# zachdedoo13/compute_path_tracer

Hardware: AMD Instinct MI355X
Metric: Msamples/sec at 1920×1080×8-bounce; achieved HBM GB/s vs gfx950 peak (higher is better)
Workload: dtype f32; 1 GPU; c3 1920x1080, 8 bounces, 256 spp per step (256 per GPU-share), progressive accumulate; width=1920, height=1080, bounces=8, parallelism=tiles1, pipelines=2, bin_samples=536870912, bin_fallback=False

## Files before the change

compute_path_tracer_amd/csrc/pt_binned.h:

```cpp
#pragma once

#include "pt_path.h"

#ifndef PT_BIN_BITS
#define PT_BIN_BITS 12
#endif
#define PT_BINS (1 << PT_BIN_BITS)
#define PT_BIN_NONE 0xffffffffu
#define PT_AUX_MISS 0xffffffffu
#define PT_BIN_BLOCK 256
#ifndef PT_RUN_SHARDS
#define PT_RUN_SHARDS 8
#endif
#define PT_CTRL_CURSOR(k) (32u * (1u + uint32_t(k)))
#define PT_CTRL_STRIDE (32u * (1u + uint32_t(PT_RUN_SHARDS)))
#ifndef PT_SCATTER_ITEMS
#define PT_SCATTER_ITEMS 16
#endif

struct PtRay {
    uint4 q[4];
};

struct PtPass {
    PtLaunch L;
    PtRay *rin;
    PtRay *rout;
    uint4 *hq;
    uint2 *mask_hi;
    uint32_t *key;
    uint32_t *idx;
    uint32_t *hist;
    uint32_t *offs;
    uint32_t *ctrl;
    const uint32_t *n_src;
    float4 *color;
    float4 *hitn;
    unsigned long long *btab;
    int32_t lanes;
    uint32_t n_src_const;
    int32_t bounce;
    int32_t n_pix;
    int32_t frames;
    int32_t wide;
    int32_t run_max;
    int32_t refill_min;
    int32_t gen_order;
    int32_t gen_trace;
    int32_t count_overflow;
    int32_t gen_norec;
};

namespace pt {

__device__ __forceinline__ uint32_t bin_hash(const uint4 &m) {
    const uint32_t h = (m.x * 0x9E3779B1u) ^ (m.y * 0x85EBCA77u) ^ (m.z * 0xC2B2AE3Du) ^ (m.w * 0x27D4EB2Fu);
    return (h ^ (h >> 15)) * 0x2C1B3C6Du >> (32 - PT_BIN_BITS);
}

#ifndef PT_BIN_PROBES
#define PT_BIN_PROBES 8
#endif
struct BinProbe {
    uint32_t h;
    unsigned long long e;
    unsigned long long v;
};
__device__ __forceinline__ BinProbe bin_probe(const PtPass &P, const uint4 &m) {
    BinProbe b;
    b.h = bin_hash(m);
    b.e = 0ull;
    b.v = 0ull;
    if (P.btab) {
        b.e = ((unsigned long long)m.y << 32 | m.x) + 1ull;
        if (b.e != 0ull) b.v = P.btab[b.h];
    }
    return b;
}
__device__ __forceinline__ uint32_t bin_resolve(const PtPass &P, const uint4 &m, BinProbe b) {
    if (!P.btab) {
        if ((m.y | m.z | m.w) == 0u && m.x < uint32_t(PT_BINS)) return m.x;
        return b.h;
    }
    if (b.e == 0ull || b.v == b.e) return b.h;
    uint32_t s = b.h;
    unsigned long long v = b.v;
    for (int k = 0;;) {
        if (v == 0ull) v = atomicCAS(P.btab + s, 0ull, b.e);
        if (v == 0ull || v == b.e) return s;
        if (++k == PT_BIN_PROBES) {
            if (P.count_overflow) atomicAdd(P.btab + PT_BINS, 1ull);
            return b.h;
        }
        s = (s + 1u) & uint32_t(PT_BINS - 1);
        v = P.btab[s];
    }
}

template <bool ST>
__device__ __forceinline__ uint4 bounds_mask(const PtLaunch &L, const pt_f3 &ro, const pt_f3 &rd, Stats<ST> &st) {
    uint32_t w[4] = {0u, 0u, 0u, 0u};
    const caabb_ptr boxes = (caabb_ptr)L.aabbs;
    const bool fast = L.fast_bounds != 0 && pt_div_coord_ok(ro.x) && pt_div_coord_ok(ro.y) &&
                      pt_div_coord_ok(ro.z) && pt_div_dir_ok(rd.x) && pt_div_dir_ok(rd.y) && pt_div_dir_ok(rd.z);
    if (fast) {
        if constexpr (ST)
            if (first_active_lane()) st.add(PT_ST_BOUNDS_WAVES);
        const float yx = 1.0f / rd.x, yy = 1.0f / rd.y, yz = 1.0f / rd.z;
        uint32_t gapu = 0xffffffffu;
#pragma unroll 4
        for (int b = 0; b < L.n_aabb; ++b) {
            const PtAabb bx = boxes[b];
            if (ray_box_ulp<false>(bx, ro.x, ro.y, ro.z, yx, yy, yz, gapu)) w[bx.back >> 5] |= 1u << (bx.back & 31);
        }
        if (__builtin_expect(__ballot(!(gapu > PT_ULP_MARGIN)) != 0ull, 0)) {
            if constexpr (ST)
                if (first_active_lane()) st.add(PT_ST_BOUNDS_EXACT);
            uint32_t v[4] = {0u, 0u, 0u, 0u};
            for (int b = 0; b < L.n_aabb; ++b) {
                const PtAabb bx = boxes[b];
                if (ray_box_rcp(bx, ro.x, ro.y, ro.z, rd.x, rd.y, rd.z, yx, yy, yz))
                    v[bx.back >> 5] |= 1u << (bx.back & 31);
            }
            if (!(gapu > PT_ULP_MARGIN))
                for (int k = 0; k < 4; ++k) w[k] = v[k];
        }
    } else {
        for (int b = 0; b < L.n_aabb; ++b) {
            const PtAabb bx = boxes[b];
            if (ray_box(bx, ro.x, ro.y, ro.z, rd.x, rd.y, rd.z)) w[bx.back >> 5] |= 1u << (bx.back & 31);
        }
    }
    st.add(PT_ST_SEGMENTS);
    st.add(PT_ST_AABB, uint32_t(L.n_aabb));
    return make_uint4(w[0], w[1], w[2], w[3]);
}

template <class Map>
struct MapWide {
    static constexpr int v = -1;
};
template <class Map>
__device__ __forceinline__ bool wide_of(const PtPass &P) {
    if constexpr (MapWide<Map>::v >= 0) return MapWide<Map>::v != 0;
    else return P.wide != 0;
}

template <class Map>
struct MapMats {
    static constexpr int n = 0;
};

template <class Map>
struct MapBounds {
    template <bool ST>
    static __device__ __forceinline__ uint4 mask(const PtLaunch &L, const pt_f3 &ro, const pt_f3 &rd, Stats<ST> &st) {
        return bounds_mask<ST>(L, ro, rd, st);
    }
    template <bool ST>
    static __device__ __forceinline__ uint4 mask_skip(const PtLaunch &L, const pt_f3 &ro, const pt_f3 &rd, uint64_t skip,
                                                      Stats<ST> &st) {
        (void)skip;
        return bounds_mask<ST>(L, ro, rd, st);
    }
};

__device__ __forceinline__ uint64_t primary_box_skip(const PtLaunch &L, const pt_f3 &ro, const pt_f3 &rd) {
    const int nb = L.n_aabb;
    if (L.fast_bounds == 0 || nb <= 0 || nb > 64) return 0ull;
    if (__builtin_amdgcn_read_exec() != ~0ull) return 0ull;
    const bool fast = pt_div_coord_ok(ro.x) && pt_div_coord_ok(ro.y) && pt_div_coord_ok(ro.z) &&
                      pt_div_dir_ok(rd.x) && pt_div_dir_ok(rd.y) && pt_div_dir_ok(rd.z);
    const uint64_t fm = __ballot(fast);
    if (fm == 0ull) return 0ull;
    const int l0 = __builtin_ctzll(fm);
    const float ox = __int_as_float(__builtin_amdgcn_readlane(__float_as_int(ro.x), l0));
    const float oy = __int_as_float(__builtin_amdgcn_readlane(__float_as_int(ro.y), l0));
    const float oz = __int_as_float(__builtin_amdgcn_readlane(__float_as_int(ro.z), l0));
    if (__ballot(fast && (__float_as_uint(ro.x) != __float_as_uint(ox) || __float_as_uint(ro.y) != __float_as_uint(oy) ||
                          __float_as_uint(ro.z) != __float_as_uint(oz))) != 0ull)
        return 0ull;
    const float inf = __builtin_inff();
    const uint32_t lane = threadIdx.x & 63u;
    const bool mine = lane < uint32_t(nb);
    static_assert(sizeof(PtAabb) == 32, "box stride");
    uint32_t off;
    __asm__ volatile("v_lshlrev_b32 %0, 5, %1" : "=v"(off) : "v"(lane));
    const float *box = reinterpret_cast<const float *>(reinterpret_cast<const char *>(L.aabbs) + off);
    float lo = -inf, hi = inf;
    auto axis = [&](int a, float d, float o) {
        const float y = 1.0f / d;
        const float ylo = wave_min_f32(fast ? y : inf), yhi = wave_max_f32(fast ? y : -inf);
        if (mine && (ylo > 0.0f || yhi < 0.0f)) {
            const float c1 = box[a] - o, c2 = box[3 + a] - o;
            const float p1 = c1 * ylo, p2 = c1 * yhi, p3 = c2 * ylo, p4 = c2 * yhi;
            lo = pt_gmax(lo, pt_gmin(pt_gmin(p1, p2), pt_gmin(p3, p4)));
            hi = pt_gmin(hi, pt_gmax(pt_gmax(p1, p2), pt_gmax(p3, p4)));
        }
    };
    axis(0, rd.x, ox);
    axis(1, rd.y, oy);
    axis(2, rd.z, oz);
    const bool skip = mine && (hi <= 0.0f ||
                               (lo > 0.0f && hi > 0.0f && __float_as_uint(lo) > __float_as_uint(hi) + PT_ULP_MARGIN));
    return __ballot(skip);
}

__device__ __forceinline__ void store_ray(PtRay *r, const pt_f3 &ro, const pt_f3 &rd, const pt_f3 &thr, uint32_t rng,
                                          uint32_t sid, uint32_t aux, const uint4 &q3) {
    r->q[0] = make_uint4(__float_as_uint(ro.x), __float_as_uint(ro.y), __float_as_uint(ro.z), __float_as_uint(rd.x));
    r->q[1] = make_uint4(__float_as_uint(rd.y), __float_as_uint(rd.z), __float_as_uint(thr.x), __float_as_uint(thr.y));
    r->q[2] = make_uint4(__float_as_uint(thr.z), rng, sid, aux);
    r->q[3] = q3;
}

__device__ __forceinline__ void hist_zero(uint32_t *lh) {
    for (int b = int(threadIdx.x); b < PT_BINS; b += int(blockDim.x)) lh[b] = 0u;
    __syncthreads();
}
__device__ __forceinline__ void hist_flush(const uint32_t *lh, uint32_t *hist) {
    __syncthreads();
    for (int b = int(threadIdx.x); b < PT_BINS; b += int(blockDim.x))
        if (lh[b] != 0u) atomicAdd(&hist[b], lh[b]);
}
__device__ __forceinline__ void pixel_of(int rank, int nranks, int tiles_x, uint32_t pl, int &x, int &y) {
    const int k = int(pl >> 6), p = int(pl & 63u);
    const int g = rank + k * nranks;
    x = (g % tiles_x) * PT_TILE + (p & 7);
    y = (g / tiles_x) * PT_TILE + (p >> 3);
}
__device__ __forceinline__ void pixel_of(const PtLaunch &L, uint32_t pl, int &x, int &y) {
    pixel_of(L.rank, L.nranks, L.tiles_x, pl, x, y);
}
__device__ __forceinline__ void gen_sample(uint32_t frames, uint32_t p, uint32_t &f, uint32_t &pl) {
    pl = p / frames;
    f = p - pl * frames;
}
__device__ __forceinline__ uint32_t colour_slot(uint32_t frames, uint32_t f, uint32_t pl) { return pl * frames + f; }

template <class Map, bool ST, int CAM = PT_CAMK_ANY>
__device__ __forceinline__ void bin_gen_body(const PtPass &P) {
    __shared__ uint32_t lh[PT_BINS];
    hist_zero(lh);
    Stats<ST> st;
    st.init();
    const PtLaunch &L = P.L;
    const uint32_t npix = uint32_t(P.n_pix), n = npix * uint32_t(P.frames);
    for (uint32_t i = blockIdx.x * blockDim.x + threadIdx.x; i < n; i += gridDim.x * blockDim.x) {
        const uint32_t f = i / npix, pl = i - f * npix;
        int x, y;
        pixel_of(L, pl, x, y);
        const bool live = x < L.width && y < L.height;
        if (P.gen_order) P.idx[i] = i;
        if (!live) {
            if (!P.gen_order) P.key[i] = PT_BIN_NONE;
            continue;
        }
        uint32_t rng;
        pt_f3 ro, rd;
        camera_ray<CAM>(x, y, int32_t(uint32_t(L.frame0) + f), L.width, L.height, L.aspect, L.fov, L.cam_mode, L.cam,
                        rng, ro, rd);
        st.add(PT_ST_SAMPLES);
        const uint4 m = MapBounds<Map>::template mask<ST>(L, ro, rd, st);
        const BinProbe bp = P.gen_order ? BinProbe{0u, 0ull, 0ull} : bin_probe(P, m);
        const uint32_t sid = colour_slot(uint32_t(P.frames), f, pl);
        store_ray(P.rin + i, ro, rd, pt_f3{1.0f, 1.0f, 1.0f}, rng, sid, i, make_uint4(m.x, m.y, 0u, 0u));
        P.color[sid] = make_float4(0.0f, 0.0f, 0.0f, 0.0f);
        if (wide_of<Map>(P)) P.mask_hi[i] = make_uint2(m.z, m.w);
        if (!P.gen_order) {
            const uint32_t b = bin_resolve(P, m, bp);
            P.key[i] = b;
            atomicAdd(&lh[b], 1u);
        }
    }
    if (!P.gen_order) hist_flush(lh, P.hist);
    flush_stats<ST>(L, st);
}

template <class Map, bool ST, bool TAPS, int CAM = PT_CAMK_ANY>
__device__ __forceinline__ void bin_shade_body(const PtPass &P) {
    __shared__ uint32_t lh[PT_BINS];
    constexpr int NM = MapMats<Map>::n;
    __shared__ PtMat lm[NM > 0 ? NM : 1];
    const PtMat *mats = P.L.mats;
    if constexpr (NM > 0) {
        const uint4 *src = reinterpret_cast<const uint4 *>(P.L.mats);
        uint4 *dst = reinterpret_cast<uint4 *>(lm);
        for (int k = int(threadIdx.x); k < NM * int(sizeof(PtMat) / 16); k += int(blockDim.x)) dst[k] = src[k];
        mats = lm;
    }
    hist_zero(lh);
    Stats<ST> st;
    st.init();
    Stats<ST> stt;
    stt.init();
    const PtLaunch &L = P.L;
    const uint32_t n = P.n_src ? *P.n_src : P.n_src_const;
    auto shade_one = [&](uint32_t i, const uint4 &q0, const uint4 &q1, const uint4 &q2, const uint4 &q3,
                         const uint2 &hi, const uint4 &hq) {
        pt_f3 ro{__uint_as_float(q0.x), __uint_as_float(q0.y), __uint_as_float(q0.z)};
        pt_f3 rd{__uint_as_float(q0.w), __uint_as_float(q1.x), __uint_as_float(q1.y)};
        pt_f3 thr{__uint_as_float(q1.z), __uint_as_float(q1.w), __uint_as_float(q2.x)};
        pt_f3 ret{0.0f, 0.0f, 0.0f};
        uint32_t rng = q2.y;
        const uint32_t sid = q2.z;
        const int mat = int(TAPS ? q2.w : hq.y);
        int seg = P.bounce;
        float dv0 = __uint_as_float(q3.x), dv1 = __uint_as_float(q3.y), dv2 = __uint_as_float(q3.z);
        if constexpr (!TAPS) {
            const float t = __uint_as_float(hq.x);
            ro = pt_f3{ro.x + rd.x * t, ro.y + rd.y * t, ro.z + rd.z * t};
            Check ck{uint64_t(q3.x) | (uint64_t(q3.y) << 32), uint64_t(hi.x) | (uint64_t(hi.y) << 32)};
            const float bnd = __uint_as_float(hq.z);
            const float bndw = bnd + (0x1.a3ap-13f + 0x1p-20f * (fabsf(ro.x) + fabsf(ro.y) + fabsf(ro.z)));
            uint64_t live = 0ull;
            float dp = 0.0f;
#pragma unroll 1
            for (int k = 0; k < 6; ++k) {
                float qx, qy, qz;
                map_point(ST_NORMAL, k, ro, rd, 0.0f, qx, qy, qz);
                if constexpr (ST)
                    if (first_active_lane()) stt.add(PT_ST_WAVE_MAPS);
                const Hit h = k == 0 ? Map::template first<ST>(L, qx, qy, qz, ck, bnd, bndw, live, stt)
                                     : Map::template rest<ST>(L, qx, qy, qz, ck, bnd, bndw, live, stt);
                if (k == 0) ck.alo = Map::alive(live);
                if ((k & 1) == 0) {
                    dp = h.d;
                } else {
                    const float dd = dp - h.d;
                    if (k == 1) dv0 = dd;
                    else if (k == 3) dv1 = dd;
                    else dv2 = dd;
                }
            }
            stt.add(PT_ST_NORMAL_MAPS, 6);
        }
        const bool done = shade_lane<ST>(mats, L.bounces, mat, dv0, dv1, dv2, 0, rng, ro, rd, thr, ret, seg, st);
        if (P.bounce == 0) st.add(PT_ST_SHADED_FIRST);
        if (P.gen_trace) {
            P.color[sid] = make_float4(ret.x, ret.y, ret.z, 0.0f);
        } else if (ret.x != 0.0f || ret.y != 0.0f || ret.z != 0.0f) {
            float4 c = P.color[sid];
            c.x += ret.x;
            c.y += ret.y;
            c.z += ret.z;
            P.color[sid] = c;
        }
        if (done) {
            if (L.debug == 3) {
                const pt_f3 col = final_color(L.debug, seg, L.bounces, ret);
                P.color[sid] = make_float4(col.x, col.y, col.z, 0.0f);
            }
            P.key[i] = PT_BIN_NONE;
            return;
        }
        const uint4 m = MapBounds<Map>::template mask<ST>(L, ro, rd, st);
        const BinProbe bp = bin_probe(P, m);
        store_ray(P.rout + i, ro, rd, thr, rng, sid, i, make_uint4(m.x, m.y, 0u, 0u));
        if (wide_of<Map>(P)) P.mask_hi[i] = make_uint2(m.z, m.w);
        const uint32_t k = bin_resolve(P, m, bp);
        P.key[i] = k;
        atomicAdd(&lh[k], 1u);
    };
    for (uint32_t i = blockIdx.x * blockDim.x + threadIdx.x; i < n; i += gridDim.x * blockDim.x) {
        if constexpr (TAPS) {
            const uint4 q0 = P.rout[i].q[0], q1 = P.rout[i].q[1], q2 = P.rout[i].q[2], q3 = P.rout[i].q[3];
            if (q2.w == PT_AUX_MISS) P.key[i] = PT_BIN_NONE;
            else shade_one(i, q0, q1, q2, q3, make_uint2(0u, 0u), q3);
        } else {
            uint4 hq = P.hq[i];
            __asm__ volatile("" : "+v"(hq.x), "+v"(hq.y), "+v"(hq.z), "+v"(hq.w));
            if (hq.y == PT_AUX_MISS) {
                P.key[i] = PT_BIN_NONE;
                continue;
            }
            uint4 q0, q1, q2, q3;
            if (P.gen_norec) {
                uint32_t npix = uint32_t(P.n_pix), nf = uint32_t(P.frames);
                int rk = L.rank, nr = L.nranks, tx = L.tiles_x, cw = L.width, chh = L.height;
                float ca = L.aspect, cf = L.fov;
                __asm__ volatile("" : "+s"(npix), "+s"(nf), "+s"(rk), "+s"(nr), "+s"(tx), "+s"(cw), "+s"(chh),
                                 "+s"(ca), "+s"(cf));
                uint32_t f, pl;
                gen_sample(nf, i, f, pl);
                int x, y;
                pixel_of(rk, nr, tx, pl, x, y);
                uint32_t rg;
                pt_f3 o, d;
                camera_ray<CAM>(x, y, int32_t(uint32_t(L.frame0) + f), cw, chh, ca, cf, L.cam_mode, L.cam, rg, o, d);
                q0 = make_uint4(__float_as_uint(o.x), __float_as_uint(o.y), __float_as_uint(o.z), __float_as_uint(d.x));
                q1 = make_uint4(__float_as_uint(d.y), __float_as_uint(d.z), __float_as_uint(1.0f), __float_as_uint(1.0f));
                q2 = make_uint4(__float_as_uint(1.0f), rg, colour_slot(nf, f, pl), i);
                q3 = make_uint4(hq.w, 0u, 0u, 0u);
            } else {
                const PtRay *r = P.rin + hq.w;
                q0 = r->q[0];
                q1 = r->q[1];
                q2 = r->q[2];
                q3 = r->q[3];
            }
            uint2 hi = make_uint2(0u, 0u);
            if (wide_of<Map>(P)) {
                const float4 nd = P.hitn[i];
                hi = make_uint2(__float_as_uint(nd.z), __float_as_uint(nd.w));
            }
            shade_one(i, q0, q1, q2, q3, hi, hq);
        }
    }
    hist_flush(lh, P.hist);
    flush_stats<ST>(L, st);
    if constexpr (!TAPS) flush_stats<ST>(L, stt, PT_ST_COUNT);
}

#define PT_SCAN_THREADS 64
__device__ __forceinline__ void bin_scan_body(const PtPass &P) {
    constexpr int PER = PT_BINS / PT_SCAN_THREADS;
    const int t = int(threadIdx.x);
    uint4 *h4 = reinterpret_cast<uint4 *>(P.hist + t * PER);
    uint4 *o4 = reinterpret_cast<uint4 *>(P.offs + t * PER);
    uint32_t sum = 0u;
#pragma unroll
    for (int j = 0; j < PER / 4; ++j) {
        const uint4 v = h4[j];
        sum += v.x + v.y + v.z + v.w;
    }
    uint32_t inc = sum;
#pragma unroll
    for (int off = 1; off < PT_SCAN_THREADS; off <<= 1) {
        const uint32_t x = uint32_t(__shfl_up(int(inc), off, PT_SCAN_THREADS));
        if (t >= off) inc += x;
    }
    uint32_t run = inc - sum;
#pragma unroll
    for (int j = 0; j < PER / 4; ++j) {
        const uint4 v = h4[j];
        uint4 o;
        o.x = run;
        run += v.x;
        o.y = run;
        run += v.y;
        o.z = run;
        run += v.z;
        o.w = run;
        run += v.w;
        o4[j] = o;
        h4[j] = make_uint4(0u, 0u, 0u, 0u);
    }
    if (t == PT_SCAN_THREADS - 1) P.ctrl[0] = inc;
    if (t < PT_RUN_SHARDS) P.ctrl[PT_CTRL_CURSOR(t)] = 0u;
}

__device__ __forceinline__ void bin_scatter_body(const PtPass &P) {
    __shared__ uint32_t cnt[PT_BINS];
    const uint32_t n = P.n_src ? *P.n_src : P.n_src_const;
    const uint32_t per = ((n + gridDim.x - 1u) / gridDim.x + PT_BIN_BLOCK - 1u) & ~uint32_t(PT_BIN_BLOCK - 1);
    const uint32_t b0 = min(n, blockIdx.x * per), b1 = min(n, b0 + per);
    constexpr uint32_t U = 8u;
    hist_zero(cnt);
    for (uint32_t e0 = b0 + threadIdx.x; e0 < b1; e0 += U * PT_BIN_BLOCK) {
        uint32_t k[U];
#pragma unroll
        for (uint32_t j = 0; j < U; ++j) {
            const uint32_t e = e0 + j * PT_BIN_BLOCK;
            k[j] = e < b1 ? P.key[e] : PT_BIN_NONE;
        }
#pragma unroll
        for (uint32_t j = 0; j < U; ++j)
            if (k[j] != PT_BIN_NONE) atomicAdd(&cnt[k[j]], 1u);
    }
    __syncthreads();
    for (int b = int(threadIdx.x); b < PT_BINS; b += PT_BIN_BLOCK) {
        const uint32_t c = cnt[b];
        if (c != 0u) cnt[b] = atomicAdd(&P.offs[b], c);
    }
    __syncthreads();
    for (uint32_t e0 = b0 + threadIdx.x; e0 < b1; e0 += U * PT_BIN_BLOCK) {
        uint32_t k[U];
#pragma unroll
        for (uint32_t j = 0; j < U; ++j) {
            const uint32_t e = e0 + j * PT_BIN_BLOCK;
            k[j] = e < b1 ? P.key[e] : PT_BIN_NONE;
        }
#pragma unroll
        for (uint32_t j = 0; j < U; ++j)
            if (k[j] != PT_BIN_NONE) P.idx[atomicAdd(&cnt[k[j]], 1u)] = e0 + j * PT_BIN_BLOCK;
    }
}

template <class Map, bool ST, bool TAPS = true, bool GEN = false, int CAM = PT_CAMK_ANY>
__device__ __forceinline__ void bin_trace_body(const PtPass &P) {
    __shared__ uint4 W[MapWide<Map>::v == 0 ? 4 : 5][64];
    const PtLaunch &L = P.L;
    const int lane = int(threadIdx.x);
    Stats<ST> st;
    st.init();
    const uint64_t t_start = st.clk();
    const uint32_t n = P.ctrl[0];
    const uint32_t rmax = uint32_t(P.run_max);
    uint32_t R = n / (gridDim.x * 8u);
    R = R < 64u ? 64u : (R > rmax ? rmax : (R + 63u) & ~63u);
    uint32_t shard = blockIdx.x % PT_RUN_SHARDS, tried = 0u;
    auto shard_lo = [&](uint32_t k) -> uint32_t {
        return k >= PT_RUN_SHARDS ? n : uint32_t((uint64_t(n >> 6) * k / PT_RUN_SHARDS) << 6);
    };
    auto take = [&](uint32_t len, uint32_t &end) -> uint32_t {
        while (tried < PT_RUN_SHARDS) {
            const uint32_t lo = shard_lo(shard), hi = shard_lo(shard + 1u);
            const uint32_t b = lo + atomicAdd(&P.ctrl[PT_CTRL_CURSOR(shard)], len);
            if (b < hi) {
                end = b + len < hi ? b + len : hi;
                return b;
            }
            shard = (shard + 1u) % PT_RUN_SHARDS;
            ++tried;
        }
        end = n;
        return n;
    };

    uint32_t nxt = 0u, nxt_end = 0u;
    if (lane == 0) nxt = take(R, nxt_end);
    uint32_t run_cur = uint32_t(__builtin_amdgcn_readfirstlane(int(nxt)));
    uint32_t run_end = uint32_t(__builtin_amdgcn_readfirstlane(int(nxt_end)));
    if (lane == 0 && run_cur < n) nxt = take(R, nxt_end);
    auto next_window = [&](uint32_t &b, uint32_t &c) {
        if (run_cur >= run_end) {
            run_cur = uint32_t(__builtin_amdgcn_readfirstlane(int(nxt)));
            run_end = uint32_t(__builtin_amdgcn_readfirstlane(int(nxt_end)));
            if (lane == 0 && run_cur < n) nxt = take(R, nxt_end);
        }
        b = run_cur;
        c = run_end - run_cur < 64u ? run_end - run_cur : 64u;
        run_cur += c;
    };
    uint32_t nb = 0u, nc = 0u, nslot = 0u;
    next_window(nb, nc);
    if (!GEN && uint32_t(lane) < nc) nslot = P.idx[nb + uint32_t(lane)];
    uint32_t wbase = 0u, wcnt = 0u, wtake = 0u;
    float4 s0 = make_float4(0.0f, 0.0f, 0.0f, 0.0f), s1 = s0, s2 = s0;
    uint4 s3 = make_uint4(0u, 0u, 0u, 0u);
    uint2 sh = make_uint2(0u, 0u);
    bool in_lds = false;
    auto stage = [&]() {
        wbase = nb;
        wcnt = nc;
        wtake = 0u;
        in_lds = false;
        if (GEN && uint32_t(lane) < wcnt) {
            const uint32_t i = wbase + uint32_t(lane), npix = uint32_t(P.n_pix);
            uint32_t f, pl;
            gen_sample(uint32_t(P.frames), i, f, pl);
            const uint32_t sid = colour_slot(uint32_t(P.frames), f, pl);
            (void)npix;
            int x, y;
            pixel_of(L, pl, x, y);
            uint32_t rg;
            pt_f3 o, d;
            float fov = L.fov;
            __asm__ volatile("" : "+v"(fov));
            camera_ray<CAM>(x, y, int32_t(uint32_t(L.frame0) + f), L.width, L.height, L.aspect, fov, L.cam_mode, L.cam,
                            rg, o, d);
            st.add(PT_ST_SAMPLES);
            const uint64_t skip = wcnt == 64u ? primary_box_skip(L, o, d) : 0ull;
            const uint4 m = MapBounds<Map>::template mask_skip<ST>(L, o, d, skip, st);
            s0 = make_float4(o.x, o.y, o.z, d.x);
            s1 = make_float4(d.y, d.z, 1.0f, 1.0f);
            s2 = make_float4(1.0f, __uint_as_float(rg), __uint_as_float(sid), __uint_as_float(i));
            s3 = make_uint4(m.x, m.y, 0u, 0u);
            sh = make_uint2(m.z, m.w);
        } else if (uint32_t(lane) < wcnt) {
            const uint32_t slot = nslot;
            const uint4 *v = reinterpret_cast<const uint4 *>(P.rin + slot);
            const uint4 a = v[0], b = v[1], c = v[2];
            s0 = make_float4(__uint_as_float(a.x), __uint_as_float(a.y), __uint_as_float(a.z), __uint_as_float(a.w));
            s1 = make_float4(__uint_as_float(b.x), __uint_as_float(b.y), __uint_as_float(b.z), __uint_as_float(b.w));
            s2 = make_float4(__uint_as_float(c.x), __uint_as_float(c.y), __uint_as_float(c.z), __uint_as_float(c.w));
            s3 = v[3];
            if (wide_of<Map>(P)) sh = P.mask_hi[slot];
        }
        if (wcnt != 0u) {
            next_window(nb, nc);
            if (!GEN && uint32_t(lane) < nc) nslot = P.idx[nb + uint32_t(lane)];
        }
    };
    stage();

    int state = ST_FREE;
    uint32_t rng = 0u, sid = 0u, pos = 0u, slot = 0u;
    pt_f3 ro{0.0f, 0.0f, 0.0f}, rd{0.0f, 0.0f, 1.0f};
    pt_f3 thr{1.0f, 1.0f, 1.0f};
    int step = 0, mat = 0;
    float t = 0.0f;
    float dv0 = 0.0f, dv1 = 0.0f, dv2 = 0.0f;
    Check ck{0ull, 0ull};

    auto hand_on = [&]() {
        if (state == ST_SHADE) {
            if (step < 0) {
                if (L.debug == 3) {
                    const pt_f3 c = final_color(L.debug, P.bounce, L.bounces, pt_f3{0.0f, 0.0f, 0.0f});
                    P.color[sid] = make_float4(c.x, c.y, c.z, 0.0f);
                }
                if constexpr (TAPS) P.rout[pos].q[2] = make_uint4(slot, 0u, sid, PT_AUX_MISS);
                else P.hq[pos] = make_uint4(0u, PT_AUX_MISS, 0u, slot);
                if constexpr (GEN) P.color[sid] = make_float4(0.0f, 0.0f, 0.0f, 0.0f);
            } else {
                if constexpr (TAPS) {
                    store_ray(P.rout + pos, ro, rd, thr, rng, sid, uint32_t(mat),
                              make_uint4(__float_as_uint(dv0), __float_as_uint(dv1), __float_as_uint(dv2), 0u));
                } else {
                    P.hq[pos] = make_uint4(__float_as_uint(t), uint32_t(mat), __float_as_uint(dv0),
                                           GEN && P.gen_norec ? uint32_t(ck.lo) : slot);
                    if (wide_of<Map>(P))
                        P.hitn[pos] = make_float4(0.0f, 0.0f, __uint_as_float(uint32_t(ck.hi)),
                                                  __uint_as_float(uint32_t(ck.hi >> 32)));
                }
            }
            state = ST_FREE;
        }
    };

    auto park = [&]() {
        const bool mapping_now = state == ST_MARCH || (TAPS && state == ST_NORMAL);
        const bool in_win = uint32_t(lane) < wcnt;
        ck.alo = wave_or_u64((mapping_now ? ck.lo : 0ull) |
                             (in_win ? (uint64_t(s3.x) | (uint64_t(s3.y) << 32)) : 0ull));
        ck.ahi = wide_of<Map>(P) ? wave_or_u64((mapping_now ? ck.hi : 0ull) |
                                      (in_win ? (uint64_t(sh.x) | (uint64_t(sh.y) << 32)) : 0ull))
                        : 0ull;
        W[0][lane] = make_uint4(__float_as_uint(s0.x), __float_as_uint(s0.y), __float_as_uint(s0.z),
                                __float_as_uint(s0.w));
        W[1][lane] = make_uint4(__float_as_uint(s1.x), __float_as_uint(s1.y), __float_as_uint(s1.z),
                                __float_as_uint(s1.w));
        W[2][lane] = make_uint4(__float_as_uint(s2.x), __float_as_uint(s2.y), __float_as_uint(s2.z),
                                __float_as_uint(s2.w));
        W[3][lane] = s3;
        if constexpr (MapWide<Map>::v != 0)
            if (wide_of<Map>(P)) W[4][lane] = make_uint4(sh.x, sh.y, 0u, 0u);
        if constexpr (GEN) {
            if (in_win && !P.gen_norec) {
                uint4 *r = reinterpret_cast<uint4 *>(P.rin + wbase + uint32_t(lane));
                r[0] = make_uint4(__float_as_uint(s0.x), __float_as_uint(s0.y), __float_as_uint(s0.z),
                                  __float_as_uint(s0.w));
                r[1] = make_uint4(__float_as_uint(s1.x), __float_as_uint(s1.y), __float_as_uint(s1.z),
                                  __float_as_uint(s1.w));
                r[2] = make_uint4(__float_as_uint(s2.x), __float_as_uint(s2.y), __float_as_uint(s2.z),
                                  __float_as_uint(s2.w));
                r[3] = s3;
            }
        }
        in_lds = true;
        __builtin_amdgcn_fence(__ATOMIC_RELEASE, "wavefront");
        __builtin_amdgcn_wave_barrier();
        __builtin_amdgcn_fence(__ATOMIC_ACQUIRE, "wavefront");
    };

    for (;;) {
        uint64_t tm = st.clk();
        const uint64_t freem = __ballot(state == ST_FREE);
        if (freem != 0ull && wcnt != 0u &&
            (__popcll(freem) >= P.refill_min || __ballot(state == ST_MARCH || state == ST_NORMAL) == 0ull)) {
            const uint32_t avail = wcnt - wtake, nf = uint32_t(__popcll(freem));
            const uint32_t take = nf < avail ? nf : avail;
            const int r = lane_rank(freem);
            const int src = int(wtake) + r;
            const bool got = state == ST_FREE && uint32_t(r) < take;
            if (!in_lds) park();
            float a0 = 0.0f, a1 = 0.0f, a2 = 0.0f, a3 = 0.0f, b0 = 0.0f, b1 = 0.0f, b2 = 0.0f, b3 = 0.0f;
            float c0 = 0.0f, c1 = 0.0f, c2 = 0.0f, c3 = 0.0f;
            uint32_t d0 = 0u, d1 = 0u, d2 = 0u, d3 = 0u, e0 = 0u, e1 = 0u;
            if (got) {
                const uint4 wa = W[0][src], wb = W[1][src], wc = W[2][src], wd = W[3][src];
                a0 = __uint_as_float(wa.x), a1 = __uint_as_float(wa.y), a2 = __uint_as_float(wa.z);
                a3 = __uint_as_float(wa.w);
                b0 = __uint_as_float(wb.x), b1 = __uint_as_float(wb.y), b2 = __uint_as_float(wb.z);
                b3 = __uint_as_float(wb.w);
                c0 = __uint_as_float(wc.x), c1 = __uint_as_float(wc.y), c2 = __uint_as_float(wc.z);
                c3 = __uint_as_float(wc.w);
                d0 = wd.x, d1 = wd.y, d2 = wd.z, d3 = wd.w;
                if constexpr (MapWide<Map>::v != 0) {
                    if (wide_of<Map>(P)) {
                        const uint4 we = W[4][src];
                        e0 = we.x;
                        e1 = we.y;
                    }
                }
            }
            if (got) {
                ro = pt_f3{a0, a1, a2};
                rd = pt_f3{a3, b0, b1};
                thr = pt_f3{b2, b3, c0};
                rng = __float_as_uint(c1);
                sid = __float_as_uint(c2);
                slot = __float_as_uint(c3);
                ck.lo = uint64_t(d0) | (uint64_t(d1) << 32);
                (void)d2;
                (void)d3;
                ck.hi = uint64_t(e0) | (uint64_t(e1) << 32);
                pos = wbase + uint32_t(src);
                t = 0.0f;
                step = 0;
                state = ST_MARCH;
            }
            wtake += take;
            if (wtake == wcnt) stage();
        }
        const bool more = wcnt != 0u;
        tm = st.lap(PT_ST_CYC_REFILL, tm);

        const bool mapping = state == ST_MARCH || (TAPS && state == ST_NORMAL);
        st.add(PT_ST_LANE_IDLE, mapping ? 0u : 1u);
        st.add(PT_ST_IDLE_SHADE, state == ST_SHADE ? 1u : 0u);
        st.add(PT_ST_IDLE_FREE, state == ST_FREE ? 1u : 0u);
        if (lane == 0) st.add(PT_ST_WAVE_ITERS);
        if (__ballot(mapping) != 0ull) {
            if (lane == 0) st.add(PT_ST_WAVE_MAPS);
            if (mapping) {
                float qx, qy, qz;
                map_point(TAPS ? state : int(ST_MARCH), step, ro, rd, t, qx, qy, qz);
                uint64_t live = 0;
                const Hit h = Map::template eval<ST>(L, qx, qy, qz, ck, __builtin_inff(), __builtin_inff(), live, st);
                after_map<ST, !TAPS>(h, state, step, t, ro, rd, mat, dv0, dv1, dv2, st);
                if constexpr (!TAPS) {
                    if (state == ST_NORMAL) {
                        dv0 = tap_bound(h.d, qx, qy, qz, t, L.bound_k);
                        state = ST_SHADE;
                    }
                }
            }
        }
        tm = st.lap(PT_ST_CYC_MAP, tm);

        hand_on();
        tm = st.lap(PT_ST_CYC_SHADE, tm);
        if (!more && __ballot(state != ST_FREE) == 0ull) break;
    }
    (void)st.lap(PT_ST_CYC_TOTAL, t_start);
    flush_stats<ST>(L, st);
}

#define PT_FOLD_SLICE 8
__device__ __forceinline__ void bin_fold_body(const PtPass &P) {
    __shared__ float4 tile[PT_BIN_BLOCK][PT_FOLD_SLICE + 1];
    const PtLaunch &L = P.L;
    const uint32_t t = threadIdx.x, pl0 = blockIdx.x * PT_BIN_BLOCK, pl = pl0 + t;
    const uint32_t npix = uint32_t(P.n_pix), fr = uint32_t(P.frames);
    const uint32_t nl = uint32_t(P.lanes > 0 ? P.lanes : 1);
    int x = 0, y = 0;
    bool mine = pl < npix && L.write;
    if (mine) {
        pixel_of(L, pl, x, y);
        mine = x < L.width && y < L.height;
    }
    float4 *texel = mine ? reinterpret_cast<float4 *>(L.accum + (size_t(y) * size_t(L.width) + size_t(x)) * 4) : nullptr;
    if (L.debug != 0) {
        if (mine) {
            const float4 c = P.color[pl];
            *texel = make_float4(c.x, c.y, c.z, 1.0f);
        }
        return;
    }
    float ar = 0.0f, ag = 0.0f, ab = 0.0f;
    if (mine) {
        const float4 v = *texel;
        ar = v.x;
        ag = v.y;
        ab = v.z;
    }
    uint32_t f0 = 0u;
    for (uint32_t j = 0u; j < nl; ++j) {
        const uint32_t fl = fr / nl + (j < fr % nl ? 1u : 0u);
        const float4 *reg = P.color + size_t(f0) * npix;
        for (uint32_t s0 = 0u; s0 < fl; s0 += PT_FOLD_SLICE) {
            const uint32_t sn = fl - s0 < PT_FOLD_SLICE ? fl - s0 : PT_FOLD_SLICE;
            __syncthreads();
            for (uint32_t e = t; e < PT_BIN_BLOCK * PT_FOLD_SLICE; e += PT_BIN_BLOCK) {
                const uint32_t q = e / PT_FOLD_SLICE, k = e % PT_FOLD_SLICE;
                if (k < sn && pl0 + q < npix) tile[q][k] = reg[size_t(pl0 + q) * fl + s0 + k];
            }
            __syncthreads();
            if (mine) {
                for (uint32_t k = 0u; k < sn; ++k) {
                    const float4 c = tile[t][k];
                    const int32_t lc = int32_t(uint32_t(L.last_clear0) + f0 + s0 + k);
                    const float w = 1.0f / float(lc + 1), omw = 1.0f - w;
                    ar = ar * omw + c.x * w;
                    ag = ag * omw + c.y * w;
                    ab = ab * omw + c.z * w;
                }
            }
        }
        f0 += fl;
    }
    if (mine) *texel = make_float4(ar, ag, ab, 1.0f);
}

}
```

compute_path_tracer_amd/csrc/pt_path.h:

```cpp
#pragma once

#include "pt_common.h"

namespace pt {

enum : int { ST_FREE = 0, ST_BOUNDS = 1, ST_MARCH = 2, ST_NORMAL = 3, ST_SHADE = 4 };

#define PT_CAMK_ANY (-1)
#define PT_CAMK_FIXED 0
#define PT_CAMK_POSED 1

template <int CAM = PT_CAMK_ANY>
__device__ __forceinline__ void camera_ray(int x, int y, int32_t frame, int width, int height, float aspect, float fov,
                                           int cam_mode, const pt_camera &cam, uint32_t &rng, pt_f3 &ro, pt_f3 &rd) {
    rng = pt_gen_rng(x, y, frame, width, height);
    float jx = pt_random01(rng);
    float jy = pt_random01(rng);
    jx = jx - 0.5f;
    jy = jy - 0.5f;
    float ux = (float(x) + jx) / float(width), uy = (float(y) + jy) / float(height);
    ux = ux * 2.0f - 1.0f;
    uy = uy * 2.0f - 1.0f;
    ux *= aspect;
    if (CAM == PT_CAMK_FIXED || (CAM == PT_CAMK_ANY && cam_mode == PT_CAM_DEFAULT)) {
        rd = pt_normalize(pt_f3{ux, uy, fov});
        ro = pt_f3{0.0f, 0.0f, -3.0f};
        return;
    }
    const float *org = cam.origin, *right = cam.right, *up = cam.up, *fwd = cam.forward;
    rd = pt_normalize(pt_f3{(right[0] * ux + up[0] * uy) + fwd[0] * fov, (right[1] * ux + up[1] * uy) + fwd[1] * fov,
                            (right[2] * ux + up[2] * uy) + fwd[2] * fov});
    ro = pt_f3{org[0], org[1], org[2]};
    if (cam_mode == PT_CAM_LENS) {
        const float aperture = cam.aperture, focus = cam.focus;
        const float u1 = pt_random01(rng);
        const float u2 = pt_random01(rng);
        const float r = pt_sqrt(u1) * aperture;
        const float a = u2 * kPi2;
        float sa, ca;
        pt_sincos(a, sa, ca);
        const float lx = r * ca, ly = r * sa;
        const pt_f3 pf{ro.x + rd.x * focus, ro.y + rd.y * focus, ro.z + rd.z * focus};
        ro = pt_f3{(ro.x + right[0] * lx) + up[0] * ly, (ro.y + right[1] * lx) + up[1] * ly,
                   (ro.z + right[2] * lx) + up[2] * ly};
        rd = pt_normalize(pt_f3{pf.x - ro.x, pf.y - ro.y, pf.z - ro.z});
    }
}

__device__ __forceinline__ pt_f3 sky_radiance(const pt_sky &sky, const pt_f3 &rd) {
    const float t = rd.y * 0.5f + 0.5f;
    pt_f3 g{sky.bottom[0] + (sky.top[0] - sky.bottom[0]) * t, sky.bottom[1] + (sky.top[1] - sky.bottom[1]) * t,
            sky.bottom[2] + (sky.top[2] - sky.bottom[2]) * t};
    const float s = pt_dot(rd, pt_f3{sky.sun_dir[0], sky.sun_dir[1], sky.sun_dir[2]});
    if (s >= sky.sun_cos) {
        g.x = g.x + sky.sun_color[0];
        g.y = g.y + sky.sun_color[1];
        g.z = g.z + sky.sun_color[2];
    }
    return g;
}

__device__ __forceinline__ void sky_miss(const PtLaunch &L, const pt_f3 &rd, const pt_f3 &thr, pt_f3 &ret) {
    if (L.sky_mode == PT_SKY_OFF) return;
    uint32_t off = uint32_t(__builtin_offsetof(PtLaunch, sky));
    __asm__ volatile("" : "+s"(off));
    const pt_sky &sky = *reinterpret_cast<const pt_sky *>(reinterpret_cast<const char *>(&L) + off);
    const pt_f3 g = sky_radiance(sky, rd);
    ret.x = ret.x + g.x * thr.x;
    ret.y = ret.y + g.y * thr.y;
    ret.z = ret.z + g.z * thr.z;
}

__device__ __forceinline__ bool ray_box(const PtAabb &bx, float ox, float oy, float oz, float dx, float dy, float dz) {
    const float tminx = (bx.bmin[0] - ox) / dx, tmaxx = (bx.bmax[0] - ox) / dx;
    const float tminy = (bx.bmin[1] - oy) / dy, tmaxy = (bx.bmax[1] - oy) / dy;
    const float tminz = (bx.bmin[2] - oz) / dz, tmaxz = (bx.bmax[2] - oz) / dz;
    const float tnear = pt_gmax(pt_gmax(pt_gmin(tminx, tmaxx), pt_gmin(tminy, tmaxy)), pt_gmin(tminz, tmaxz));
    const float tfar = pt_gmin(pt_gmin(pt_gmax(tminx, tmaxx), pt_gmax(tminy, tmaxy)), pt_gmax(tminz, tmaxz));
    return tnear < tfar && tfar > 0.0f;
}

__device__ __forceinline__ bool ray_box_rcp(const PtAabb &bx, float ox, float oy, float oz, float dx, float dy,
                                            float dz, float yx, float yy, float yz) {
    const float tminx = pt_div_rcp(bx.bmin[0] - ox, dx, yx), tmaxx = pt_div_rcp(bx.bmax[0] - ox, dx, yx);
    const float tminy = pt_div_rcp(bx.bmin[1] - oy, dy, yy), tmaxy = pt_div_rcp(bx.bmax[1] - oy, dy, yy);
    const float tminz = pt_div_rcp(bx.bmin[2] - oz, dz, yz), tmaxz = pt_div_rcp(bx.bmax[2] - oz, dz, yz);
    const float tnear = pt_gmax(pt_gmax(pt_gmin(tminx, tmaxx), pt_gmin(tminy, tmaxy)), pt_gmin(tminz, tmaxz));
    const float tfar = pt_gmin(pt_gmin(pt_gmax(tminx, tmaxx), pt_gmax(tminy, tmaxy)), pt_gmax(tminz, tmaxz));
    return tnear < tfar && tfar > 0.0f;
}

__device__ __forceinline__ bool ray_box_approx(const PtAabb &bx, float ox, float oy, float oz, float yx, float yy,
                                               float yz, float &gap) {
    const float tminx = (bx.bmin[0] - ox) * yx, tmaxx = (bx.bmax[0] - ox) * yx;
    const float tminy = (bx.bmin[1] - oy) * yy, tmaxy = (bx.bmax[1] - oy) * yy;
    const float tminz = (bx.bmin[2] - oz) * yz, tmaxz = (bx.bmax[2] - oz) * yz;
    const float tnear = pt_gmax(pt_gmax(pt_gmin(tminx, tmaxx), pt_gmin(tminy, tmaxy)), pt_gmin(tminz, tmaxz));
    const float tfar = pt_gmin(pt_gmin(pt_gmax(tminx, tmaxx), pt_gmax(tminy, tmaxy)), pt_gmax(tminz, tmaxz));
    gap = fminf(gap, fabsf(tfar - tnear) - (fabsf(tnear) + fabsf(tfar)) * 0x1p-20f);
    return tnear < tfar && tfar > 0.0f;
}

#define PT_ULP_MARGIN 16u
template <bool SAD = true>
__device__ __forceinline__ uint32_t pt_absdiff_u32(uint32_t a, uint32_t b) {
    if constexpr (!SAD) return max(a, b) - min(a, b);
    uint32_t d;
    __asm__("v_sad_u32 %0, %1, %2, 0" : "=v"(d) : "v"(a), "v"(b));
    return d;
}
template <bool SAD = true>
__device__ __forceinline__ bool ray_box_ulp(const PtAabb &bx, float ox, float oy, float oz, float yx, float yy,
                                            float yz, uint32_t &gapu) {
    const float tminx = (bx.bmin[0] - ox) * yx, tmaxx = (bx.bmax[0] - ox) * yx;
    const float tminy = (bx.bmin[1] - oy) * yy, tmaxy = (bx.bmax[1] - oy) * yy;
    const float tminz = (bx.bmin[2] - oz) * yz, tmaxz = (bx.bmax[2] - oz) * yz;
    const float tnear = pt_gmax(pt_gmax(pt_gmin(tminx, tmaxx), pt_gmin(tminy, tmaxy)), pt_gmin(tminz, tmaxz));
    const float tfar = pt_gmin(pt_gmin(pt_gmax(tminx, tmaxx), pt_gmax(tminy, tmaxy)), pt_gmax(tminz, tmaxz));
    gapu = min(gapu, pt_absdiff_u32<SAD>(__float_as_uint(tfar), __float_as_uint(tnear)));
    return tnear < tfar && tfar > 0.0f;
}

__device__ __forceinline__ bool ray_box_fma(const PtAabb &bx, float nx, float ny, float nz, float yx, float yy,
                                            float yz, float &gap, float &tfa) {
    const float tminx = fmaf(bx.bmin[0], yx, nx), tmaxx = fmaf(bx.bmax[0], yx, nx);
    const float tminy = fmaf(bx.bmin[1], yy, ny), tmaxy = fmaf(bx.bmax[1], yy, ny);
    const float tminz = fmaf(bx.bmin[2], yz, nz), tmaxz = fmaf(bx.bmax[2], yz, nz);
    const float tnear = pt_gmax(pt_gmax(pt_gmin(tminx, tmaxx), pt_gmin(tminy, tmaxy)), pt_gmin(tminz, tmaxz));
    const float tfar = pt_gmin(pt_gmin(pt_gmax(tminx, tmaxx), pt_gmax(tminy, tmaxy)), pt_gmax(tminz, tmaxz));
    gap = fminf(gap, fabsf(tfar - tnear) - (fabsf(tnear) + fabsf(tfar)) * 0x1p-20f);
    tfa = fminf(tfa, fabsf(tfar));
    return tnear < tfar && tfar > 0.0f;
}
__device__ __forceinline__ bool fma_decided(float gap, float tfa, float nx, float ny, float nz) {
    const float m = pt_gmax(fabsf(nx), pt_gmax(fabsf(ny), fabsf(nz)));
    return gap > m * 0x1p-21f && tfa > m * 0x1p-22f;
}

__device__ __forceinline__ void map_point(int state, int step, const pt_f3 &ro, const pt_f3 &rd, float t, float &qx,
                                          float &qy, float &qz) {
    if (state == ST_MARCH) {
        qx = ro.x + rd.x * t;
        qy = ro.y + rd.y * t;
        qz = ro.z + rd.z * t;
    } else {
        const float e = 0.0001f;
        const int axis = step >> 1;
        const bool neg = (step & 1) != 0;
        const float on = neg ? -e : e, off = neg ? -0.0f : 0.0f;
        qx = ro.x + (axis == 0 ? on : off);
        qy = ro.y + (axis == 1 ? on : off);
        qz = ro.z + (axis == 2 ? on : off);
    }
}

template <bool ST, bool MARCH_ONLY = false>
__device__ __forceinline__ void after_map(const Hit &h, int &state, int &step, float &t, pt_f3 &ro, const pt_f3 &rd,
                                          int &mat, float &dv0, float &dv1, float &dv2, Stats<ST> &st) {
    if (MARCH_ONLY || state == ST_MARCH) {
        st.add(PT_ST_MARCH);
        mat = h.m;
        t += h.d;
        ++step;
        if (fabsf(h.d) < kMhd || t > kFp || step == kSteps) {
            if (t > kFp) {
                state = ST_SHADE;
                step = -1;
            } else {
                ro = pt_f3{ro.x + rd.x * t, ro.y + rd.y * t, ro.z + rd.z * t};
                state = ST_NORMAL;
                step = 0;
            }
        }
    } else if constexpr (!MARCH_ONLY) {
        if ((step & 1) == 0) {
            t = h.d;
        } else {
            const float dd = t - h.d;
            if (step == 1) dv0 = dd;
            else if (step == 3) dv1 = dd;
            else dv2 = dd;
        }
        ++step;
        if (step == 6) {
            st.add(PT_ST_NORMAL_MAPS, 6);
            state = ST_SHADE;
        }
    }
}

__device__ __forceinline__ float tap_bound(float d, float qx, float qy, float qz, float t, float bk) {
    const float ad = fabsf(d);
    const float mg = 0x1p-10f * (fabsf(qx) + fabsf(qy) + fabsf(qz) + ad + fabsf(t) + bk);
    return ((d + ad) * 0x1.0001p+0f + mg) + 0x1.a38p-14f;
}

template <bool ST>
__device__ __forceinline__ bool shade_lane(const PtMat *__restrict__ mats, int bounces, int mat, float dv0, float dv1,
                                           float dv2, int step, uint32_t &rng, pt_f3 &ro, pt_f3 &rd, pt_f3 &thr,
                                           pt_f3 &ret, int &seg, Stats<ST> &st) {
    if (step < 0) return true;
    const pt_f3 n = pt_normalize(pt_f3{dv0, dv1, dv2});
    const pt_f3 hp = ro;
    ro = pt_f3{hp.x + n.x * kOffset, hp.y + n.y * kOffset, hp.z + n.z * kOffset};
    st.add(PT_ST_SHADED);
    const PtMat &m = mats[mat];
    const float spec_chance = m.spec;
    const bool do_spec = pt_random01(rng) < spec_chance;
    float ray_prob = do_spec ? spec_chance : 1.0f - spec_chance;
    ray_prob = pt_gmax(ray_prob, 0.0001f);
    const float uz = pt_random01(rng) * 2.0f - 1.0f;
    const float ua = pt_random01(rng) * kPi2;
    const float ur = pt_sqrt(1.0f - uz * uz);
    float sa, ca;
    pt_sincos(ua, sa, ca);
    const pt_f3 diffuse = pt_normalize(pt_f3{n.x + ur * ca, n.y + ur * sa, n.z + uz});
    if (do_spec) {
        const float k = 2.0f * pt_dot(n, rd);
        const pt_f3 sr{rd.x - k * n.x, rd.y - k * n.y, rd.z - k * n.z};
        const float al = m.rough2, oma = 1.0f - al;
        rd = pt_normalize(pt_f3{sr.x * oma + diffuse.x * al, sr.y * oma + diffuse.y * al, sr.z * oma + diffuse.z * al});
    } else {
        rd = diffuse;
    }
    const float fs = do_spec ? 1.0f : 0.0f, omf = 1.0f - fs;
    ret.x += m.emis[0] * thr.x;
    ret.y += m.emis[1] * thr.y;
    ret.z += m.emis[2] * thr.z;
    thr.x *= m.col[0] * omf + m.spec_col[0] * fs;
    thr.y *= m.col[1] * omf + m.spec_col[1] * fs;
    thr.z *= m.col[2] * omf + m.spec_col[2] * fs;
    thr.x /= ray_prob;
    thr.y /= ray_prob;
    thr.z /= ray_prob;
    const float pmax = pt_gmax(thr.x, pt_gmax(thr.y, thr.z));
    if (pt_random01(rng) > pmax) {
        st.add(PT_ST_RR_BREAK);
        return true;
    }
    const float ip = 1.0f / pmax;
    thr.x *= ip;
    thr.y *= ip;
    thr.z *= ip;
    ++seg;
    return seg > bounces;
}

__device__ __forceinline__ pt_f3 final_color(int debug, int seg, int bounces, const pt_f3 &ret) {
    if (debug == 3) {
        const float v = float(seg) / float(bounces);
        return pt_f3{v, v, v};
    }
    return ret;
}

}
```

Measured before the change: 2868 Msamples/sec.

## Split shading into fate and bounce, skip normal taps for terminated paths

Shading is split into a fate step (RNG draws, emission, throughput, Russian roulette) and a bounce step (normal, offset, new direction). Only lanes whose path continues now run the 6-tap SDF normal estimation and direction sampling, and a wave skips it entirely when no lane needs it. On the final bounce the kernel returns right after accumulating colour, skipping the histogram, key writes and the ray store. This saves costly map evaluations for rays killed by roulette or the bounce limit, at the cost of more divergence inside waves and extra code paths.

```diff
diff --git a/compute_path_tracer_amd/csrc/pt_binned.h b/compute_path_tracer_amd/csrc/pt_binned.h
--- a/compute_path_tracer_amd/csrc/pt_binned.h
+++ b/compute_path_tracer_amd/csrc/pt_binned.h
@@ -289,12 +289,14 @@
         for (int k = int(threadIdx.x); k < NM * int(sizeof(PtMat) / 16); k += int(blockDim.x)) dst[k] = src[k];
         mats = lm;
     }
-    hist_zero(lh);
+    const PtLaunch &L = P.L;
+    const bool last = !TAPS && !ST && L.debug == 0 && P.bounce == L.bounces;
+    if (last) __syncthreads();
+    else hist_zero(lh);
     Stats<ST> st;
     st.init();
     Stats<ST> stt;
     stt.init();
-    const PtLaunch &L = P.L;
     const uint32_t n = P.n_src ? *P.n_src : P.n_src_const;
     auto shade_one = [&](uint32_t i, const uint4 &q0, const uint4 &q1, const uint4 &q2, const uint4 &q3,
                          const uint2 &hi, const uint4 &hq) {
@@ -307,44 +309,59 @@
         const int mat = int(TAPS ? q2.w : hq.y);
         int seg = P.bounce;
         float dv0 = __uint_as_float(q3.x), dv1 = __uint_as_float(q3.y), dv2 = __uint_as_float(q3.z);
-        if constexpr (!TAPS) {
+        auto emit = [&]() {
+            if (P.bounce == 0) st.add(PT_ST_SHADED_FIRST);
+            if (P.gen_trace) {
+                P.color[sid] = make_float4(ret.x, ret.y, ret.z, 0.0f);
+            } else if (ret.x != 0.0f || ret.y != 0.0f || ret.z != 0.0f) {
+                float4 c = P.color[sid];
+                c.x += ret.x;
+                c.y += ret.y;
+                c.z += ret.z;
+                P.color[sid] = c;
+            }
+        };
+        bool done;
+        if constexpr (TAPS) {
+            done = shade_lane<ST>(mats, L.bounces, mat, dv0, dv1, dv2, 0, rng, ro, rd, thr, ret, seg, st);
+            emit();
+        } else {
+            ShadeDraws sd;
+            done = shade_fate<ST>(mats, L.bounces, mat, rng, thr, ret, seg, sd, st);
+            emit();
+            if (last) return;
             const float t = __uint_as_float(hq.x);
             ro = pt_f3{ro.x + rd.x * t, ro.y + rd.y * t, ro.z + rd.z * t};
-            Check ck{uint64_t(q3.x) | (uint64_t(q3.y) << 32), uint64_t(hi.x) | (uint64_t(hi.y) << 32)};
-            const float bnd = __uint_as_float(hq.z);
-            const float bndw = bnd + (0x1.a3ap-13f + 0x1p-20f * (fabsf(ro.x) + fabsf(ro.y) + fabsf(ro.z)));
-            uint64_t live = 0ull;
-            float dp = 0.0f;
+            const bool tap = ST || L.debug != 0 || !done;
+            if (__ballot(tap) != 0ull) {
+                if (tap) {
+                    Check ck{uint64_t(q3.x) | (uint64_t(q3.y) << 32), uint64_t(hi.x) | (uint64_t(hi.y) << 32)};
+                    const float bnd = __uint_as_float(hq.z);
+                    const float bndw = bnd + (0x1.a3ap-13f + 0x1p-20f * (fabsf(ro.x) + fabsf(ro.y) + fabsf(ro.z)));
+                    uint64_t live = 0ull;
+                    float dp = 0.0f;
 #pragma unroll 1
-            for (int k = 0; k < 6; ++k) {
-                float qx, qy, qz;
-                map_point(ST_NORMAL, k, ro, rd, 0.0f, qx, qy, qz);
-                if constexpr (ST)
-                    if (first_active_lane()) stt.add(PT_ST_WAVE_MAPS);
-                const Hit h = k == 0 ? Map::template first<ST>(L, qx, qy, qz, ck, bnd, bndw, live, stt)
-                                     : Map::template rest<ST>(L, qx, qy, qz, ck, bnd, bndw, live, stt);
-                if (k == 0) ck.alo = Map::alive(live);
-                if ((k & 1) == 0) {
-                    dp = h.d;
-                } else {
-                    const float dd = dp - h.d;
-                    if (k == 1) dv0 = dd;
-                    else if (k == 3) dv1 = dd;
-                    else dv2 = dd;
+                    for (int k = 0; k < 6; ++k) {
+                        float qx, qy, qz;
+                        map_point(ST_NORMAL, k, ro, rd, 0.0f, qx, qy, qz);
+                        if constexpr (ST)
+                            if (first_active_lane()) stt.add(PT_ST_WAVE_MAPS);
+                        const Hit h = k == 0 ? Map::template first<ST>(L, qx, qy, qz, ck, bnd, bndw, live, stt)
+                                             : Map::template rest<ST>(L, qx, qy, qz, ck, bnd, bndw, live, stt);
+                        if (k == 0) ck.alo = Map::alive(live);
+                        if ((k & 1) == 0) {
+                            dp = h.d;
+                        } else {
+                            const float dd = dp - h.d;
+                            if (k == 1) dv0 = dd;
+                            else if (k == 3) dv1 = dd;
+                            else dv2 = dd;
+                        }
+                    }
+                    stt.add(PT_ST_NORMAL_MAPS, 6);
                 }
             }
-            stt.add(PT_ST_NORMAL_MAPS, 6);
-        }
-        const bool done = shade_lane<ST>(mats, L.bounces, mat, dv0, dv1, dv2, 0, rng, ro, rd, thr, ret, seg, st);
-        if (P.bounce == 0) st.add(PT_ST_SHADED_FIRST);
-        if (P.gen_trace) {
-            P.color[sid] = make_float4(ret.x, ret.y, ret.z, 0.0f);
-        } else if (ret.x != 0.0f || ret.y != 0.0f || ret.z != 0.0f) {
-            float4 c = P.color[sid];
-            c.x += ret.x;
-            c.y += ret.y;
-            c.z += ret.z;
-            P.color[sid] = c;
+            if (!done) shade_bounce(dv0, dv1, dv2, sd, ro, rd);
         }
         if (done) {
             if (L.debug == 3) {
@@ -371,7 +388,7 @@
             uint4 hq = P.hq[i];
             __asm__ volatile("" : "+v"(hq.x), "+v"(hq.y), "+v"(hq.z), "+v"(hq.w));
             if (hq.y == PT_AUX_MISS) {
-                P.key[i] = PT_BIN_NONE;
+                if (!last) P.key[i] = PT_BIN_NONE;
                 continue;
             }
             uint4 q0, q1, q2, q3;
@@ -407,7 +424,7 @@
             shade_one(i, q0, q1, q2, q3, hi, hq);
         }
     }
-    hist_flush(lh, P.hist);
+    if (!last) hist_flush(lh, P.hist);
     flush_stats<ST>(L, st);
     if constexpr (!TAPS) flush_stats<ST>(L, stt, PT_ST_COUNT);
 }
diff --git a/compute_path_tracer_amd/csrc/pt_path.h b/compute_path_tracer_amd/csrc/pt_path.h
--- a/compute_path_tracer_amd/csrc/pt_path.h
+++ b/compute_path_tracer_amd/csrc/pt_path.h
@@ -195,34 +195,29 @@
     return ((d + ad) * 0x1.0001p+0f + mg) + 0x1.a38p-14f;
 }
 
+struct ShadeDraws {
+    bool do_spec;
+    float uz, ua;
+    float rough2;
+};
+
+__device__ __forceinline__ void shade_draws(const PtMat &m, uint32_t &rng, ShadeDraws &d) {
+    d.do_spec = pt_random01(rng) < m.spec;
+    d.uz = pt_random01(rng) * 2.0f - 1.0f;
+    d.ua = pt_random01(rng) * kPi2;
+    d.rough2 = m.rough2;
+}
+
 template <bool ST>
-__device__ __forceinline__ bool shade_lane(const PtMat *__restrict__ mats, int bounces, int mat, float dv0, float dv1,
-                                           float dv2, int step, uint32_t &rng, pt_f3 &ro, pt_f3 &rd, pt_f3 &thr,
-                                           pt_f3 &ret, int &seg, Stats<ST> &st) {
-    if (step < 0) return true;
-    const pt_f3 n = pt_normalize(pt_f3{dv0, dv1, dv2});
-    const pt_f3 hp = ro;
-    ro = pt_f3{hp.x + n.x * kOffset, hp.y + n.y * kOffset, hp.z + n.z * kOffset};
+__device__ __forceinline__ bool shade_fate(const PtMat *__restrict__ mats, int bounces, int mat, uint32_t &rng,
+                                           pt_f3 &thr, pt_f3 &ret, int &seg, ShadeDraws &d, Stats<ST> &st) {
     st.add(PT_ST_SHADED);
     const PtMat &m = mats[mat];
     const float spec_chance = m.spec;
-    const bool do_spec = pt_random01(rng) < spec_chance;
+    shade_draws(m, rng, d);
+    const bool do_spec = d.do_spec;
     float ray_prob = do_spec ? spec_chance : 1.0f - spec_chance;
     ray_prob = pt_gmax(ray_prob, 0.0001f);
-    const float uz = pt_random01(rng) * 2.0f - 1.0f;
-    const float ua = pt_random01(rng) * kPi2;
-    const float ur = pt_sqrt(1.0f - uz * uz);
-    float sa, ca;
-    pt_sincos(ua, sa, ca);
-    const pt_f3 diffuse = pt_normalize(pt_f3{n.x + ur * ca, n.y + ur * sa, n.z + uz});
-    if (do_spec) {
-        const float k = 2.0f * pt_dot(n, rd);
-        const pt_f3 sr{rd.x - k * n.x, rd.y - k * n.y, rd.z - k * n.z};
-        const float al = m.rough2, oma = 1.0f - al;
-        rd = pt_normalize(pt_f3{sr.x * oma + diffuse.x * al, sr.y * oma + diffuse.y * al, sr.z * oma + diffuse.z * al});
-    } else {
-        rd = diffuse;
-    }
     const float fs = do_spec ? 1.0f : 0.0f, omf = 1.0f - fs;
     ret.x += m.emis[0] * thr.x;
     ret.y += m.emis[1] * thr.y;
@@ -246,6 +241,37 @@
     return seg > bounces;
 }
 
+__device__ __forceinline__ void shade_bounce(float dv0, float dv1, float dv2, const ShadeDraws &d, pt_f3 &ro,
+                                             pt_f3 &rd) {
+    const pt_f3 n = pt_normalize(pt_f3{dv0, dv1, dv2});
+    const pt_f3 hp = ro;
+    ro = pt_f3{hp.x + n.x * kOffset, hp.y + n.y * kOffset, hp.z + n.z * kOffset};
+    const float uz = d.uz, ua = d.ua;
+    const float ur = pt_sqrt(1.0f - uz * uz);
+    float sa, ca;
+    pt_sincos(ua, sa, ca);
+    const pt_f3 diffuse = pt_normalize(pt_f3{n.x + ur * ca, n.y + ur * sa, n.z + uz});
+    if (d.do_spec) {
+        const float k = 2.0f * pt_dot(n, rd);
+        const pt_f3 sr{rd.x - k * n.x, rd.y - k * n.y, rd.z - k * n.z};
+        const float al = d.rough2, oma = 1.0f - al;
+        rd = pt_normalize(pt_f3{sr.x * oma + diffuse.x * al, sr.y * oma + diffuse.y * al, sr.z * oma + diffuse.z * al});
+    } else {
+        rd = diffuse;
+    }
+}
+
+template <bool ST>
+__device__ __forceinline__ bool shade_lane(const PtMat *__restrict__ mats, int bounces, int mat, float dv0, float dv1,
+                                           float dv2, int step, uint32_t &rng, pt_f3 &ro, pt_f3 &rd, pt_f3 &thr,
+                                           pt_f3 &ret, int &seg, Stats<ST> &st) {
+    if (step < 0) return true;
+    ShadeDraws d;
+    const bool done = shade_fate<ST>(mats, bounces, mat, rng, thr, ret, seg, d, st);
+    shade_bounce(dv0, dv1, dv2, d, ro, rd);
+    return done;
+}
+
 __device__ __forceinline__ pt_f3 final_color(int debug, int seg, int bounces, const pt_f3 &ret) {
     if (debug == 3) {
         const float v = float(seg) / float(bounces);
```

Result: no change. 2882 Msamples/sec, median of 6 (+0.5%).
